# CVPR23/Depth-guided-Texture-Diffusion-for-Image-Semantic-Segmentation

Measured on NVIDIA B200. Metric: rgbd_images_per_sec_384, higher is better.
Workload: dtype bf16

## Files before the change

depth-guided-texture-diffusion-for-image-semantic-segmentation_b200/csrc/blackwell.cuh:

```cuda
#pragma once
#include <cuda.h>
#include <cuda_runtime.h>
#include <stdint.h>
#include <stdio.h>

namespace dgtd {
namespace bw {

__device__ __forceinline__ uint32_t smem_u32(const void* p) {
  return static_cast<uint32_t>(__cvta_generic_to_shared(p));
}

__device__ __forceinline__ bool elect_one() {
  uint32_t pred = 0;
  asm volatile(
      "{\n\t.reg .pred p;\n\t"
      "elect.sync _|p, 0xffffffff;\n\t"
      "selp.u32 %0, 1, 0, p;\n\t}"
      : "=r"(pred));
  return pred != 0;
}

__device__ __forceinline__ void mbar_init(uint64_t* bar, uint32_t count) {
  asm volatile("mbarrier.init.shared::cta.b64 [%0], %1;" ::"r"(smem_u32(bar)), "r"(count));
// ... 155 lines not shown
  asm volatile(
      "tcgen05.ld.sync.aligned.32x32b.x32.b32 "
      "{%0, %1, %2, %3, %4, %5, %6, %7, %8, %9, %10, %11, %12, %13, %14, %15, "
      "%16, %17, %18, %19, %20, %21, %22, %23, %24, %25, %26, %27, %28, %29, %30, %31}, [%32];"
      : "=r"(v[0]), "=r"(v[1]), "=r"(v[2]), "=r"(v[3]), "=r"(v[4]), "=r"(v[5]), "=r"(v[6]), "=r"(v[7]),
        "=r"(v[8]), "=r"(v[9]), "=r"(v[10]), "=r"(v[11]), "=r"(v[12]), "=r"(v[13]), "=r"(v[14]),
        "=r"(v[15]), "=r"(v[16]), "=r"(v[17]), "=r"(v[18]), "=r"(v[19]), "=r"(v[20]), "=r"(v[21]),
        "=r"(v[22]), "=r"(v[23]), "=r"(v[24]), "=r"(v[25]), "=r"(v[26]), "=r"(v[27]), "=r"(v[28]),
        "=r"(v[29]), "=r"(v[30]), "=r"(v[31])
      : "r"(taddr)
      : "memory");
}
__device__ __forceinline__ void tmem_ld_wait() { asm volatile("tcgen05.wait::ld.sync.aligned;" ::: "memory"); }

__device__ __forceinline__ uint64_t umma_smem_desc_kmajor(uint32_t smem_addr, uint32_t row_bytes) {
  const uint64_t layout = row_bytes == 128 ? 2ull : row_bytes == 64 ? 4ull : 6ull;
  return (uint64_t)((smem_addr >> 4) & 0x3FFF) | ((uint64_t)((8 * row_bytes) >> 4) << 32) |
         (1ull << 46) | (layout << 61);
}
__device__ __forceinline__ uint64_t umma_smem_desc_mnmajor_sw128(uint32_t smem_addr, uint32_t lbo_bytes,
                                                                 uint32_t sbo_bytes) {
  return (uint64_t)((smem_addr >> 4) & 0x3FFF) | ((uint64_t)((lbo_bytes >> 4) & 0x3FFF) << 16) |
         ((uint64_t)((sbo_bytes >> 4) & 0x3FFF) << 32) | (1ull << 46) | (2ull << 61);
}
__host__ __device__ constexpr uint32_t umma_idesc_bf16(int M, int N) {
  return (1u << 4) | (1u << 7) | (1u << 10) | ((uint32_t)(N >> 3) << 17) | ((uint32_t)(M >> 4) << 24);
}
__host__ __device__ constexpr uint32_t umma_idesc_tf32(int M, int N) {
  return (1u << 4) | (2u << 7) | (2u << 10) | ((uint32_t)(N >> 3) << 17) | ((uint32_t)(M >> 4) << 24);
}

}

typedef CUresult (*PFN_tmapEncodeTiled)(CUtensorMap*, CUtensorMapDataType, cuuint32_t, void*,
                                        const cuuint64_t*, const cuuint64_t*, const cuuint32_t*,
                                        const cuuint32_t*, CUtensorMapInterleave, CUtensorMapSwizzle,
                                        CUtensorMapL2promotion, CUtensorMapFloatOOBfill);
PFN_tmapEncodeTiled get_tmap_encoder();

int make_tmap(CUtensorMap* out, const void* base, CUtensorMapDataType dt, int rank,
              const uint64_t* dims, const uint64_t* strides_bytes, const uint32_t* box,
              CUtensorMapSwizzle swz);

}
```

depth-guided-texture-diffusion-for-image-semantic-segmentation_b200/csrc/mlp_fused.cu:

```cuda
#include "tc_common.cuh"

namespace dgtd {

namespace mlpf {

constexpr int C = 128, HID = 4 * C, HC = 128, NCH = HID / HC;
constexpr int BLK = 128 * 64 * 2;
constexpr int KB1 = C / 64, KB2 = HC / 64;
constexpr int A_BYTES = KB1 * BLK, H_BYTES = KB2 * BLK;
constexpr int WST = 4;
constexpr int NEPI = 16;
constexpr int STG_BYTES = NEPI * 4096;
constexpr int OFF_A = 0, OFF_H = A_BYTES, OFF_W = OFF_H + 2 * H_BYTES, OFF_STG = OFF_W + WST * BLK, OFF_BAR = OFF_STG + STG_BYTES;
constexpr int NBARS = 2 + 2 * WST + 4 + 4 + 4 + NEPI;
constexpr int SMEM = OFF_BAR + NBARS * 8 + 16;
constexpr int THREADS = 128 + NEPI * 32;
static_assert(SMEM <= 232448, "shared memory budget");

struct Params {
  const float* row_stats;
  const float* col_s;
  const float* cbias;
  const float* b2;
  const float* gamma;
  const float* res;
  float* out;
  int M, tiles;
};

__device__ __forceinline__ uint32_t swz_l(int lane) { return (uint32_t)(lane & 7); }

__global__ void __launch_bounds__(THREADS, 1)
mlp_fused_kernel(const __grid_constant__ CUtensorMap tmY, const __grid_constant__ CUtensorMap tmW1,
                 const __grid_constant__ CUtensorMap tmW2, const __grid_constant__ CUtensorMap tmRes,
                 const __grid_constant__ CUtensorMap tmOut, const Params p) {
  extern __shared__ __align__(1024) uint8_t smem[];
  uint8_t* sA = smem + OFF_A;
  uint8_t* sH = smem + OFF_H;
  uint8_t* sW = smem + OFF_W;
  uint64_t* bars = reinterpret_cast<uint64_t*>(smem + OFF_BAR);
  uint8_t* sStg = smem + OFF_STG;
  uint64_t* a_full = bars;
  uint64_t* a_empty = a_full + 1;
  uint64_t* w_full = a_empty + 1;
  uint64_t* w_empty = w_full + WST;
  uint64_t* c1_full = w_empty + WST;
  uint64_t* c1_empty = c1_full + 2;
  uint64_t* h_full = c1_empty + 2;
  uint64_t* h_empty = h_full + 2;
  uint64_t* c2_full = h_empty + 2;
  uint64_t* c2_empty = c2_full + 2;
  uint64_t* r_full = c2_empty + 2;
  uint32_t* tmem_slot = reinterpret_cast<uint32_t*>(r_full + NEPI);

  const int warp = threadIdx.x >> 5, lane = threadIdx.x & 31;
  if (warp == 0 && lane == 0) {
    bw::prefetch_tmap(&tmY);
    bw::prefetch_tmap(&tmW1);
    bw::prefetch_tmap(&tmW2);
    bw::prefetch_tmap(&tmRes);
    bw::prefetch_tmap(&tmOut);
  }
  if (warp == 1 && lane == 0) {
    bw::mbar_init(a_full, 1);
    bw::mbar_init(a_empty, 1);
    for (int i = 0; i < 2; ++i) {
      bw::mbar_init(&c1_full[i], 1);
      bw::mbar_init(&c1_empty[i], NEPI);
      bw::mbar_init(&h_full[i], NEPI);
      bw::mbar_init(&h_empty[i], 1);
      bw::mbar_init(&c2_full[i], 1);
      bw::mbar_init(&c2_empty[i], NEPI);
    }
    for (int i = 0; i < NEPI; ++i) bw::mbar_init(&r_full[i], 1);
    for (int i = 0; i < WST; ++i) {
      bw::mbar_init(&w_full[i], 1);
      bw::mbar_init(&w_empty[i], 1);
    }
    bw::fence_mbar_init();
  }
  if (warp == 2) bw::tmem_alloc(tmem_slot, 512);
  bw::tc_fence_before();
  __syncthreads();
  bw::tc_fence_after();
  const uint32_t tmem_base = *tmem_slot;

  if (warp == 0) {
    if (lane == 0) {
      int ws = 0;
      uint32_t wph = 0;
      auto load_w = [&](const CUtensorMap* tm, int k0, int r0) {
        bw::mbar_wait(&w_empty[ws], wph ^ 1);
        bw::mbar_arrive_expect_tx(&w_full[ws], BLK);
        bw::tma_load_2d(tm, &w_full[ws], sW + ws * BLK, k0, r0);
        if (++ws == WST) { ws = 0; wph ^= 1; }
      };
      int it = 0;
      for (int tile = blockIdx.x; tile < p.tiles; tile += gridDim.x, ++it) {
        bw::mbar_wait(a_empty, (it & 1) ^ 1);
        bw::mbar_arrive_expect_tx(a_full, A_BYTES);
        for (int kb = 0; kb < KB1; ++kb) bw::tma_load_2d(&tmY, a_full, sA + kb * BLK, kb * 64, tile * 128);
        for (int s = 0; s <= NCH; ++s) {
          if (s < NCH)
            for (int kb = 0; kb < KB1; ++kb) load_w(&tmW1, kb * 64, s * HC);
          if (s >= 1)
            for (int kb = 0; kb < KB2; ++kb) load_w(&tmW2, (s - 1) * HC + kb * 64, 0);
        }
      }
    }
  } else if (warp == 1) {
    if (lane == 0) {
      constexpr uint32_t idesc = bw::umma_idesc_bf16(128, 128);
      int ws = 0;
      uint32_t wph = 0;
      uint32_t q1 = 0, q2 = 0;
      int it = 0;
      for (int tile = blockIdx.x; tile < p.tiles; tile += gridDim.x, ++it) {
        const int ab = it & 1;
        bw::mbar_wait(a_full, it & 1);
        for (int s = 0; s <= NCH; ++s) {
          if (s < NCH) {
            const uint32_t b = q1 & 1;
            bw::mbar_wait(&c1_empty[b], ((q1 >> 1) & 1) ^ 1);
            bw::tc_fence_after();
            const uint32_t d = tmem_base + b * HC;
            for (int kb = 0; kb < KB1; ++kb) {
              bw::mbar_wait(&w_full[ws], wph);
              bw::tc_fence_after();
              const uint64_t da = bw::umma_smem_desc_kmajor(bw::smem_u32(sA + kb * BLK), 128);
              const uint64_t db = bw::umma_smem_desc_kmajor(bw::smem_u32(sW + ws * BLK), 128);
#pragma unroll
              for (int k = 0; k < 4; ++k) bw::umma_bf16(d, da + 2 * k, db + 2 * k, idesc, (kb | k) != 0);
              bw::umma_commit(&w_empty[ws]);
              if (++ws == WST) { ws = 0; wph ^= 1; }
            }
            bw::umma_commit(&c1_full[b]);
            if (s == NCH - 1) bw::umma_commit(a_empty);
            ++q1;
          }
          if (s >= 1) {
            const int c = s - 1;
            const uint32_t b = q2 & 1;
            if (c == 0) {
              bw::mbar_wait(&c2_empty[ab], ((it >> 1) & 1) ^ 1);
              bw::tc_fence_after();
            }
            bw::mbar_wait(&h_full[b], (q2 >> 1) & 1);
            bw::tc_fence_after();
            const uint32_t d = tmem_base + 2 * HC + ab * C;
            for (int kb = 0; kb < KB2; ++kb) {
              bw::mbar_wait(&w_full[ws], wph);
              bw::tc_fence_after();
              const uint64_t da = bw::umma_smem_desc_kmajor(bw::smem_u32(sH + b * H_BYTES + kb * BLK), 128);
              const uint64_t db = bw::umma_smem_desc_kmajor(bw::smem_u32(sW + ws * BLK), 128);
#pragma unroll
              for (int k = 0; k < 4; ++k) bw::umma_bf16(d, da + 2 * k, db + 2 * k, idesc, (c | kb | k) != 0);
              bw::umma_commit(&w_empty[ws]);
              if (++ws == WST) { ws = 0; wph ^= 1; }
            }
            bw::umma_commit(&h_empty[b]);
            if (c == NCH - 1) bw::umma_commit(&c2_full[ab]);
            ++q2;
          }
        }
      }
    }
  } else if (warp >= 4) {
    const int quad = warp & 3, part = (warp - 4) >> 2, ew = warp - 4;
    const int r = quad * 32 + lane;
    const uint32_t lane_addr = (uint32_t)(quad * 32) << 16;
    uint8_t* hrow_p = sH + (part >> 1) * BLK + r * 128;
    const uint32_t swz = (uint32_t)(r & 7);
    uint8_t* stg = sStg + ew * 4096;
    uint8_t* srow_p = stg + lane * 128;
    uint64_t* rbar = &r_full[ew];
    uint32_t q = 0;
    int it = 0;
    for (int tile = blockIdx.x; tile < p.tiles; tile += gridDim.x, ++it) {
      const int ab = it & 1;
      const int row0 = tile * 128 + quad * 32;
      if (lane == 0) {
        bw::tma_store_wait_read<0>();
        bw::mbar_arrive_expect_tx(rbar, 4096);
        bw::tma_load_2d(&tmRes, rbar, stg, part * 32, row0);
      }
      const float2 rs = __ldg(reinterpret_cast<const float2*>(p.row_stats) + row0 + lane);
      const uint64_t nm = pk2(-rs.x, -rs.x), rr = pk2(rs.y, rs.y);
      for (int c = 0; c < NCH; ++c, ++q) {
        const uint32_t b = q & 1;
        bw::mbar_wait(&c1_full[b], (q >> 1) & 1);
        bw::tc_fence_after();
        uint32_t v[32];
        bw::tmem_ld_32x32(tmem_base + lane_addr + b * HC + part * 32, v);
        bw::tmem_ld_wait();
        bw::tc_fence_before();
        __syncwarp();
        if (lane == 0) bw::mbar_arrive(&c1_empty[b]);
        bw::mbar_wait(&h_empty[b], ((q >> 1) & 1) ^ 1);
        const int n0 = c * HC + part * 32;
#pragma unroll
        for (int j = 0; j < 32; j += 8) {
          const float4 s0 = __ldg(reinterpret_cast<const float4*>(p.col_s + n0 + j));
          const float4 s1 = __ldg(reinterpret_cast<const float4*>(p.col_s + n0 + j + 4));
          const float4 b0 = __ldg(reinterpret_cast<const float4*>(p.cbias + n0 + j));
          const float4 b1 = __ldg(reinterpret_cast<const float4*>(p.cbias + n0 + j + 4));
          float f[8];
#pragma unroll
          for (int e = 0; e < 8; ++e) f[e] = __uint_as_float(v[j + e]);
          uint64_t x0 = fma2(nm, pk2(s0.x, s0.y), pk2(f[0], f[1])), x1 = fma2(nm, pk2(s0.z, s0.w), pk2(f[2], f[3]));
          uint64_t x2 = fma2(nm, pk2(s1.x, s1.y), pk2(f[4], f[5])), x3 = fma2(nm, pk2(s1.z, s1.w), pk2(f[6], f[7]));
          up2(fma2(rr, x0, pk2(b0.x, b0.y)), f[0], f[1]);
          up2(fma2(rr, x1, pk2(b0.z, b0.w)), f[2], f[3]);
          up2(fma2(rr, x2, pk2(b1.x, b1.y)), f[4], f[5]);
          up2(fma2(rr, x3, pk2(b1.z, b1.w)), f[6], f[7]);
#pragma unroll
          for (int e = 0; e < 8; e += 2) DGTD_GELU2(f[e], f[e + 1]);
          const __nv_bfloat162 a0 = __floats2bfloat162_rn(f[0], f[1]), a1 = __floats2bfloat162_rn(f[2], f[3]);
          const __nv_bfloat162 a2 = __floats2bfloat162_rn(f[4], f[5]), a3 = __floats2bfloat162_rn(f[6], f[7]);
          const uint32_t ch = (uint32_t)((part & 1) * 4 + (j >> 3));
          *reinterpret_cast<uint4*>(hrow_p + b * H_BYTES + ((ch ^ swz) << 4)) =
              make_uint4(*reinterpret_cast<const uint32_t*>(&a0), *reinterpret_cast<const uint32_t*>(&a1),
                         *reinterpret_cast<const uint32_t*>(&a2), *reinterpret_cast<const uint32_t*>(&a3));
        }
        bw::fence_proxy_async_smem();
        __syncwarp();
        if (lane == 0) bw::mbar_arrive(&h_full[b]);
      }
      bw::mbar_wait(&c2_full[ab], (it >> 1) & 1);
      bw::tc_fence_after();
      uint32_t v[32];
      bw::tmem_ld_32x32(tmem_base + lane_addr + 2 * HC + ab * C + part * 32, v);
      bw::tmem_ld_wait();
      bw::tc_fence_before();
      __syncwarp();
      if (lane == 0) bw::mbar_arrive(&c2_empty[ab]);
      bw::mbar_wait(rbar, it & 1);
#pragma unroll
      for (int j = 0; j < 32; j += 4) {
        float4* sp = reinterpret_cast<float4*>(srow_p + ((((uint32_t)(j >> 2)) ^ swz_l(lane)) << 4));
        float4 x = *sp;
        const float4 bb = __ldg(reinterpret_cast<const float4*>(p.b2 + part * 32 + j));
        float4 g = make_float4(1.f, 1.f, 1.f, 1.f);
        if (p.gamma) g = __ldg(reinterpret_cast<const float4*>(p.gamma + part * 32 + j));
        x.x += g.x * (__uint_as_float(v[j]) + bb.x);
        x.y += g.y * (__uint_as_float(v[j + 1]) + bb.y);
        x.z += g.z * (__uint_as_float(v[j + 2]) + bb.z);
        x.w += g.w * (__uint_as_float(v[j + 3]) + bb.w);
        *sp = x;
      }
      bw::fence_proxy_async_smem();
      __syncwarp();
      if (lane == 0) {
        bw::tma_store_2d(&tmOut, stg, part * 32, row0);
        bw::tma_store_commit();
      }
    }
    if (lane == 0) bw::tma_store_wait_all<0>();
  }

  bw::tc_fence_before();
  __syncthreads();
  if (warp == 2) {
    bw::tc_fence_after();
    bw::tmem_dealloc(tmem_base, 512);
  }
}

}
}

using namespace dgtd;

extern "C" int dgtd_convnext_mlp_fused_fwd(const void* y, const float* row_stats, const void* w1, const float* col_s,
                                           const float* cbias, const void* w2, const float* b2, const float* gamma,
                                           const float* residual, float* out, int64_t M, int C, dgtd_stream_t stream) {
  using namespace mlpf;
  DGTD_CHECK_ARG(y && row_stats && w1 && col_s && cbias && w2 && b2 && residual && out, "convnext_mlp_fused: null pointer");
  DGTD_CHECK_ARG(C == mlpf::C, "convnext_mlp_fused: C = %d is not built (stage 0, C = 128, only)", C);
  DGTD_CHECK_ARG(M > 0 && M % 128 == 0 && M < ((int64_t)1 << 31), "convnext_mlp_fused: M = %lld must be a positive multiple of 128",
                 (long long)M);
  cudaStream_t s = (cudaStream_t)stream;
  CUtensorMap tmY, tmW1, tmW2;
  {
    uint64_t dims[2] = {(uint64_t)C, (uint64_t)M}, str[1] = {(uint64_t)C * 2};
    uint32_t box[2] = {64, 128};
    if (make_tmap(&tmY, y, CU_TENSOR_MAP_DATA_TYPE_BFLOAT16, 2, dims, str, box, CU_TENSOR_MAP_SWIZZLE_128B)) return -3;
  }
  {
    uint64_t dims[2] = {(uint64_t)C, (uint64_t)HID}, str[1] = {(uint64_t)C * 2};
    uint32_t box[2] = {64, 128};
    if (make_tmap(&tmW1, w1, CU_TENSOR_MAP_DATA_TYPE_BFLOAT16, 2, dims, str, box, CU_TENSOR_MAP_SWIZZLE_128B)) return -3;
  }
  {
    uint64_t dims[2] = {(uint64_t)HID, (uint64_t)C}, str[1] = {(uint64_t)HID * 2};
    uint32_t box[2] = {64, 128};
    if (make_tmap(&tmW2, w2, CU_TENSOR_MAP_DATA_TYPE_BFLOAT16, 2, dims, str, box, CU_TENSOR_MAP_SWIZZLE_128B)) return -3;
  }
  CUtensorMap tmRes, tmOut;
  {
    uint64_t dims[2] = {(uint64_t)C, (uint64_t)M}, str[1] = {(uint64_t)C * 4};
    uint32_t box[2] = {32, 32};
    if (make_tmap(&tmRes, residual, CU_TENSOR_MAP_DATA_TYPE_FLOAT32, 2, dims, str, box, CU_TENSOR_MAP_SWIZZLE_128B)) return -3;
    if (make_tmap(&tmOut, out, CU_TENSOR_MAP_DATA_TYPE_FLOAT32, 2, dims, str, box, CU_TENSOR_MAP_SWIZZLE_128B)) return -3;
  }
  static bool configured = false;
  if (!configured) {
    cudaError_t e = cudaFuncSetAttribute(mlp_fused_kernel, cudaFuncAttributeMaxDynamicSharedMemorySize, SMEM);
    if (e != cudaSuccess) {
      set_error("convnext_mlp_fused: cannot opt in to %d B of shared memory: %s", SMEM, cudaGetErrorString(e));
      return -2;
    }
    configured = true;
  }
  Params p;
  p.row_stats = row_stats; p.col_s = col_s; p.cbias = cbias; p.b2 = b2; p.gamma = gamma; p.res = residual; p.out = out;
  p.M = (int)M; p.tiles = (int)(M / 128);
  const int grid = p.tiles < sm_count() ? p.tiles : sm_count();
  mlp_fused_kernel<<<grid, THREADS, SMEM, s>>>(tmY, tmW1, tmW2, tmRes, tmOut, p);
  DGTD_LAUNCH_CHECK("convnext_mlp_fused");
  return 0;
}
```

depth-guided-texture-diffusion-for-image-semantic-segmentation_b200/csrc/tc_gemm2.cu:

```cuda
#include "tc_common.cuh"

namespace dgtd {

namespace bw2 {
__device__ __forceinline__ uint32_t cta_rank() {
  uint32_t r;
  asm volatile("mov.u32 %0, %%cluster_ctarank;" : "=r"(r));
  return r;
}
__device__ __forceinline__ void cluster_sync() {
  asm volatile("barrier.cluster.arrive.release.aligned;" ::: "memory");
  asm volatile("barrier.cluster.wait.acquire.aligned;" ::: "memory");
}
__device__ __forceinline__ uint32_t map_to_rank(const void* p, uint32_t rank) {
  uint32_t r;
  asm volatile("mapa.shared::cluster.u32 %0, %1, %2;" : "=r"(r) : "r"(bw::smem_u32(p)), "r"(rank));
  return r;
}
__device__ __forceinline__ void mbar_arrive_cluster(uint32_t cluster_addr) {
  asm volatile("mbarrier.arrive.shared::cluster.b64 _, [%0];" ::"r"(cluster_addr) : "memory");
}
__device__ __forceinline__ void tma_load_2d_2sm(const CUtensorMap* m, uint32_t leader_bar, void* dst, int c0,
                                                int c1) {
  asm volatile(
      "cp.async.bulk.tensor.2d.cta_group::2.shared::cluster.global.mbarrier::complete_tx::bytes [%0], [%1, {%3, %4}], [%2];"
      ::"r"(bw::smem_u32(dst)), "l"(reinterpret_cast<uint64_t>(m)), "r"(leader_bar), "r"(c0), "r"(c1)
      : "memory");
}
__device__ __forceinline__ void tmem_alloc_2sm(uint32_t* dst_smem, uint32_t cols) {
  asm volatile("tcgen05.alloc.cta_group::2.sync.aligned.shared::cta.b32 [%0], %1;" ::"r"(bw::smem_u32(dst_smem)),
               "r"(cols)
               : "memory");
  asm volatile("tcgen05.relinquish_alloc_permit.cta_group::2.sync.aligned;" ::: "memory");
}
__device__ __forceinline__ void tmem_dealloc_2sm(uint32_t addr, uint32_t cols) {
  asm volatile("tcgen05.dealloc.cta_group::2.sync.aligned.b32 %0, %1;" ::"r"(addr), "r"(cols) : "memory");
}
__device__ __forceinline__ void umma_bf16_2sm(uint32_t tmem_d, uint64_t da, uint64_t db, uint32_t idesc,
                                              uint32_t accumulate) {
  asm volatile(
      "{\n\t.reg .pred p;\n\t"
      "setp.ne.b32 p, %4, 0;\n\t"
      "tcgen05.mma.cta_group::2.kind::f16 [%0], %1, %2, %3, p;\n\t}"
      ::"r"(tmem_d), "l"(da), "l"(db), "r"(idesc), "r"(accumulate)
      : "memory");
}
__device__ __forceinline__ void umma_commit_2sm(uint64_t* bar) {
  asm volatile(
      "tcgen05.commit.cta_group::2.mbarrier::arrive::one.shared::cluster.multicast::cluster.b64 [%0], %1;"
      ::"r"(bw::smem_u32(bar)), "h"((uint16_t)3)
      : "memory");
}
}

template <int BN>
struct Tc2Cfg {
  static constexpr int BM = 128, BK = 64;
  static constexpr int A_BYTES = BM * BK * 2, B_BYTES = (BN / 2) * BK * 2;
  static constexpr int STAGES = BN >= 256 ? 5 : 6;
  static constexpr int TMEM_COLS = 2 * BN;
  static constexpr int STG_BYTES = 8 * 2 * 4096;
  static constexpr int XCH_BYTES = BN == 128 ? 2 * 8 * 32 * 8 : 0;
  static constexpr int SMEM_BYTES = STAGES * (A_BYTES + B_BYTES) + STG_BYTES + 512 + XCH_BYTES + 1024;
};

template <int BN, int ACT, typename OT, bool RESIDUAL, int NEPI = 8, bool LNROW = false>
__global__ void __cluster_dims__(2, 1, 1) __launch_bounds__(128 + 32 * NEPI, 1)
tc_gemm2_kernel(const __grid_constant__ CUtensorMap tmA, const __grid_constant__ CUtensorMap tmB,
                const __grid_constant__ CUtensorMap tmOut, const __grid_constant__ CUtensorMap tmRes,
                const TcParams p) {
  using Cfg = Tc2Cfg<BN>;
  constexpr int BM = Cfg::BM, BK = Cfg::BK, STAGES = Cfg::STAGES;
  extern __shared__ __align__(1024) uint8_t smem[];
  uint8_t* sA = smem;
  uint8_t* sB = smem + STAGES * Cfg::A_BYTES;
  uint8_t* sStg = smem + STAGES * (Cfg::A_BYTES + Cfg::B_BYTES);
  uint64_t* bars = reinterpret_cast<uint64_t*>(sStg + Cfg::STG_BYTES);
  uint64_t* rbars = bars + 2 * STAGES + 6;
  uint64_t* full = bars;
  uint64_t* empty = bars + STAGES;
  uint64_t* tfull = bars + 2 * STAGES;
  uint64_t* tempty = bars + 2 * STAGES + 2;
  uint32_t* tmem_slot = reinterpret_cast<uint32_t*>(bars + 2 * STAGES + 4);

  const int warp = threadIdx.x >> 5, lane = threadIdx.x & 31;
  const uint32_t rank = bw2::cta_rank();
// ... 245 lines not shown
```

depth-guided-texture-diffusion-for-image-semantic-segmentation_b200/twig/ops/functions/texture_diffusion_func.py:

```python
from __future__ import annotations

from typing import List, Optional, Sequence, Tuple

import torch
from torch.autograd import Function
from torch.autograd.function import once_differentiable

from .. import capi
from ..capi import ACT_GELU, ACT_NONE, ACT_RELU, BF16, F32, call, check_cuda, ptr, stream

__all__ = [
    "surface_normals", "HighpassPlan", "fft_highpass", "diffusion_front", "MessagePassingFunction",
    "message_passing_core", "message_passing_tiled", "conv1x1_nchw_autograd", "resize_bilinear_nchw_autograd", "conv1x1_nchw", "resize_nchw", "layer_norm",
    "stem", "stem_patches", "ln_rows_", "fusion_sum", "ln_patchify", "dwconv7_ln", "dwconv7_ln_tma", "linear", "linear_ln", "linear_tf32", "linear_residual_", "conv_nhwc", "conv_nhwc_grouped",
    "resize_nhwc", "cast", "nhwc_to_nchw", "nchw_to_nhwc", "enable_gemm_profile", "collect_gemm_profile",
]


_PROFILE = {"on": False, "events": []}


def enable_gemm_profile(on: bool = True):
    _PROFILE["on"] = bool(on)
    _PROFILE["events"] = []
# ... 351 lines not shown
    M = a.numel() // K
    N = w.shape[0]
    assert w.shape[1] == K and a.dtype == torch.bfloat16 and w.dtype == torch.bfloat16 and a.is_contiguous()
    out = torch.empty(tuple(a.shape[:-1]) + (N,), device=a.device, dtype=torch.float32)
    call("dgtd_linear_ln_fwd", ptr(a), ptr(w), ptr(bias), ptr(ln_w), ptr(ln_b), float(eps), ptr(out), M, N, K, stream())
    return out


def linear_tf32(a: torch.Tensor, w: torch.Tensor, bias: Optional[torch.Tensor]) -> torch.Tensor:
    check_cuda(a, w, bias)
    K = a.shape[-1]
    M = a.numel() // K
    N = w.shape[0]
    assert w.shape[1] == K and a.dtype == torch.float32 and w.dtype == torch.float32 and a.is_contiguous()
    out = torch.empty(tuple(a.shape[:-1]) + (N,), device=a.device, dtype=torch.float32)
    call("dgtd_linear_tf32_fwd", ptr(a), ptr(w), ptr(bias), ptr(out), M, N, K, N, stream())
    return out


def linear_residual_(a: torch.Tensor, w: torch.Tensor, bias, gamma, keep: Optional[torch.Tensor],
                     rows_per_sample: int, residual: torch.Tensor, out: Optional[torch.Tensor] = None):
    check_cuda(a, w, bias, gamma, keep, residual)
    K = a.shape[-1]
    M = a.numel() // K
    N = w.shape[0]
    assert residual.dtype == torch.float32 and residual.numel() == M * N
    out = residual if out is None else out
    with _timed(2.0 * M * N * K, a.dtype == torch.bfloat16, (M, N, K)):
        call("dgtd_linear_residual_fwd", ptr(a), ptr(w), ptr(bias), ptr(gamma), ptr(keep), rows_per_sample,
             ptr(residual), ptr(out), M, N, K, capi.dtype_code(a.dtype), stream())
    return out


MLP_FUSED_C = (128,)


def convnext_mlp_fused_(y: torch.Tensor, row_stats: torch.Tensor, w1: torch.Tensor, col_s: torch.Tensor,
                        cbias: torch.Tensor, w2: torch.Tensor, b2: torch.Tensor, gamma: Optional[torch.Tensor],
                        residual: torch.Tensor, out: Optional[torch.Tensor] = None) -> torch.Tensor:
    check_cuda(y, row_stats, w1, col_s, cbias, w2, b2, gamma, residual)
    C = y.shape[-1]
    M = y.numel() // C
    assert y.dtype == torch.bfloat16 and w1.dtype == torch.bfloat16 and w2.dtype == torch.bfloat16
    assert w1.shape == (4 * C, C) and w2.shape == (C, 4 * C) and row_stats.shape == (M, 2)
    assert residual.dtype == torch.float32 and residual.numel() == M * C
    out = residual if out is None else out
    with _timed(4.0 * M * C * 4 * C, True, (M, 4 * C, C)):
        call("dgtd_convnext_mlp_fused_fwd", ptr(y), ptr(row_stats), ptr(w1), ptr(col_s), ptr(cbias), ptr(w2), ptr(b2),
             ptr(gamma), ptr(residual), ptr(out), M, C, stream())
    return out


def fusion_sum(levels: List[torch.Tensor], hw: List[Tuple[int, int]], bias, B: int, want_nhwc=True,
               want_nchw=False, pad_to: int = 0):
    check_cuda(*levels, bias)
    C = levels[0].shape[-1]
    dev = levels[0].device
    h0, w0 = hw[0]
    nhwc = torch.empty(B, h0, w0, C, device=dev, dtype=torch.float32) if want_nhwc else None
    nchw = torch.empty(B, C, h0, w0, device=dev, dtype=torch.float32) if want_nchw else None
    pad = torch.empty(B, h0, w0, pad_to, device=dev, dtype=torch.bfloat16) if pad_to else None
    hw_arr = (capi.c_int * 8)(*[v for pair in hw for v in pair])
    call("dgtd_fusion_sum_fwd", ptr(levels[0]), ptr(levels[1]), ptr(levels[2]), ptr(levels[3]), hw_arr,
         ptr(bias), ptr(nhwc), ptr(nchw), ptr(pad), pad_to, B, C, stream())
    return nhwc, nchw, pad


# ... 82 lines not shown
```

Measured before the change: 5303.

## Convert fused ConvNeXt MLP kernel to 2-SM cluster UMMA and add C=256

Rewrites the fused ConvNeXt MLP kernel to run as 2-CTA clusters using cta_group::2 tcgen05 MMAs with M=256 tiles, splitting weight tiles across the pair of CTAs. It double-buffers the A tile and C2 accumulators for C=128 and reworks the epilogue staging and residual handling. It also templates the kernel over C and enables the fused path for C=256 stages, so more of the network uses the fused kernel. The cluster barriers and cross-CTA signalling add synchronisation complexity and carry correctness risk.

After: 5222, median of 6. -1.5%, worse.

```diff
diff --git a/depth-guided-texture-diffusion-for-image-semantic-segmentation_b200/csrc/blackwell.cuh b/depth-guided-texture-diffusion-for-image-semantic-segmentation_b200/csrc/blackwell.cuh
--- a/depth-guided-texture-diffusion-for-image-semantic-segmentation_b200/csrc/blackwell.cuh
+++ b/depth-guided-texture-diffusion-for-image-semantic-segmentation_b200/csrc/blackwell.cuh
@@ -211,6 +211,60 @@
 
 }
 
+namespace bw2 {
+__device__ __forceinline__ uint32_t cta_rank() {
+  uint32_t r;
+  asm volatile("mov.u32 %0, %%cluster_ctarank;" : "=r"(r));
+  return r;
+}
+__device__ __forceinline__ void cluster_sync() {
+  asm volatile("barrier.cluster.arrive.release.aligned;" ::: "memory");
+  asm volatile("barrier.cluster.wait.acquire.aligned;" ::: "memory");
+}
+__device__ __forceinline__ uint32_t map_to_rank(const void* p, uint32_t rank) {
+  uint32_t r;
+  asm volatile("mapa.shared::cluster.u32 %0, %1, %2;" : "=r"(r) : "r"(bw::smem_u32(p)), "r"(rank));
+  return r;
+}
+__device__ __forceinline__ void mbar_arrive_cluster(uint32_t cluster_addr) {
+  asm volatile("mbarrier.arrive.shared::cluster.b64 _, [%0];" ::"r"(cluster_addr) : "memory");
+}
+__device__ __forceinline__ void mbar_arrive_cluster_release(uint32_t cluster_addr) {
+  asm volatile("mbarrier.arrive.release.cluster.shared::cluster.b64 _, [%0];" ::"r"(cluster_addr) : "memory");
+}
+__device__ __forceinline__ void tma_load_2d_2sm(const CUtensorMap* m, uint32_t leader_bar, void* dst, int c0,
+                                                int c1) {
+  asm volatile(
+      "cp.async.bulk.tensor.2d.cta_group::2.shared::cluster.global.mbarrier::complete_tx::bytes [%0], [%1, {%3, %4}], [%2];"
+      ::"r"(bw::smem_u32(dst)), "l"(reinterpret_cast<uint64_t>(m)), "r"(leader_bar), "r"(c0), "r"(c1)
+      : "memory");
+}
+__device__ __forceinline__ void tmem_alloc_2sm(uint32_t* dst_smem, uint32_t cols) {
+  asm volatile("tcgen05.alloc.cta_group::2.sync.aligned.shared::cta.b32 [%0], %1;" ::"r"(bw::smem_u32(dst_smem)),
+               "r"(cols)
+               : "memory");
+  asm volatile("tcgen05.relinquish_alloc_permit.cta_group::2.sync.aligned;" ::: "memory");
+}
+__device__ __forceinline__ void tmem_dealloc_2sm(uint32_t addr, uint32_t cols) {
+  asm volatile("tcgen05.dealloc.cta_group::2.sync.aligned.b32 %0, %1;" ::"r"(addr), "r"(cols) : "memory");
+}
+__device__ __forceinline__ void umma_bf16_2sm(uint32_t tmem_d, uint64_t da, uint64_t db, uint32_t idesc,
+                                              uint32_t accumulate) {
+  asm volatile(
+      "{\n\t.reg .pred p;\n\t"
+      "setp.ne.b32 p, %4, 0;\n\t"
+      "tcgen05.mma.cta_group::2.kind::f16 [%0], %1, %2, %3, p;\n\t}"
+      ::"r"(tmem_d), "l"(da), "l"(db), "r"(idesc), "r"(accumulate)
+      : "memory");
+}
+__device__ __forceinline__ void umma_commit_2sm(uint64_t* bar) {
+  asm volatile(
+      "tcgen05.commit.cta_group::2.mbarrier::arrive::one.shared::cluster.multicast::cluster.b64 [%0], %1;"
+      ::"r"(bw::smem_u32(bar)), "h"((uint16_t)3)
+      : "memory");
+}
+}
+
 typedef CUresult (*PFN_tmapEncodeTiled)(CUtensorMap*, CUtensorMapDataType, cuuint32_t, void*,
                                         const cuuint64_t*, const cuuint64_t*, const cuuint32_t*,
                                         const cuuint32_t*, CUtensorMapInterleave, CUtensorMapSwizzle,
diff --git a/depth-guided-texture-diffusion-for-image-semantic-segmentation_b200/csrc/mlp_fused.cu b/depth-guided-texture-diffusion-for-image-semantic-segmentation_b200/csrc/mlp_fused.cu
--- a/depth-guided-texture-diffusion-for-image-semantic-segmentation_b200/csrc/mlp_fused.cu
+++ b/depth-guided-texture-diffusion-for-image-semantic-segmentation_b200/csrc/mlp_fused.cu
@@ -4,18 +4,31 @@
 
 namespace mlpf {
 
-constexpr int C = 128, HID = 4 * C, HC = 128, NCH = HID / HC;
-constexpr int BLK = 128 * 64 * 2;
-constexpr int KB1 = C / 64, KB2 = HC / 64;
-constexpr int A_BYTES = KB1 * BLK, H_BYTES = KB2 * BLK;
-constexpr int WST = 4;
-constexpr int NEPI = 16;
-constexpr int STG_BYTES = NEPI * 4096;
-constexpr int OFF_A = 0, OFF_H = A_BYTES, OFF_W = OFF_H + 2 * H_BYTES, OFF_STG = OFF_W + WST * BLK, OFF_BAR = OFF_STG + STG_BYTES;
-constexpr int NBARS = 2 + 2 * WST + 4 + 4 + 4 + NEPI;
-constexpr int SMEM = OFF_BAR + NBARS * 8 + 16;
-constexpr int THREADS = 128 + NEPI * 32;
-static_assert(SMEM <= 232448, "shared memory budget");
+template <int C>
+struct Cfg {
+  static constexpr int HID = 4 * C, HC = 128, NCH = HID / HC;
+  static constexpr int BLK = 128 * 64 * 2;
+  static constexpr int KB1 = C / 64, KB2 = HC / 64;
+  static constexpr int A_BYTES = KB1 * BLK, H_BYTES = KB2 * BLK;
+  static constexpr int NA = C == 128 ? 2 : 1;
+  static constexpr int NACC2 = C == 128 ? 2 : 1;
+  static constexpr int WST = 4, SLOT = 16384;
+  static constexpr int W1_HALF = 64 * 64 * 2;
+  static constexpr int W2_HALF = (C / 2) * 64 * 2;
+  static constexpr int W2_PER_SLOT = SLOT / W2_HALF;
+  static constexpr int SLOTS1 = KB1 / 2, SLOTS2 = KB2 / W2_PER_SLOT;
+  static constexpr int NEPI = 16;
+  static constexpr int CW = C / 4;
+  static constexpr int STG = 2048;
+  static constexpr int OFF_A = 0, OFF_H = NA * A_BYTES, OFF_W = OFF_H + 2 * H_BYTES, OFF_STG = OFF_W + WST * SLOT;
+  static constexpr int OFF_BAR = OFF_STG + NEPI * STG;
+  static constexpr int NBARS = 2 * NA + 2 * WST + 4 + 4 + 2 * NACC2;
+  static constexpr int SMEM = OFF_BAR + NBARS * 8 + 16;
+  static constexpr int THREADS = 128 + NEPI * 32;
+  static_assert(SMEM <= 232448, "shared memory budget");
+  static_assert(SLOTS1 * 2 == KB1 && SLOTS2 * W2_PER_SLOT == KB2, "weight blocks fill whole ring slots");
+  static_assert(2 * HC + NACC2 * C <= 512, "TMEM budget");
+};
 
 struct Params {
   const float* row_stats;
@@ -24,64 +37,69 @@
   const float* b2;
   const float* gamma;
   const float* res;
-  float* out;
   int M, tiles;
 };
 
-__device__ __forceinline__ uint32_t swz_l(int lane) { return (uint32_t)(lane & 7); }
-
-__global__ void __launch_bounds__(THREADS, 1)
+template <int C>
+__global__ void __cluster_dims__(2, 1, 1) __launch_bounds__(Cfg<C>::THREADS, 1)
 mlp_fused_kernel(const __grid_constant__ CUtensorMap tmY, const __grid_constant__ CUtensorMap tmW1,
-                 const __grid_constant__ CUtensorMap tmW2, const __grid_constant__ CUtensorMap tmRes,
-                 const __grid_constant__ CUtensorMap tmOut, const Params p) {
+                 const __grid_constant__ CUtensorMap tmW2, const __grid_constant__ CUtensorMap tmOut, const Params p) {
+  using K = Cfg<C>;
+  constexpr int HC = K::HC, NCH = K::NCH, NA = K::NA, NACC2 = K::NACC2, WST = K::WST, NEPI = K::NEPI, CW = K::CW;
   extern __shared__ __align__(1024) uint8_t smem[];
-  uint8_t* sA = smem + OFF_A;
-  uint8_t* sH = smem + OFF_H;
-  uint8_t* sW = smem + OFF_W;
-  uint64_t* bars = reinterpret_cast<uint64_t*>(smem + OFF_BAR);
-  uint8_t* sStg = smem + OFF_STG;
+  uint8_t* sA = smem + K::OFF_A;
+  uint8_t* sH = smem + K::OFF_H;
+  uint8_t* sW = smem + K::OFF_W;
+  uint8_t* sStg = smem + K::OFF_STG;
+  uint64_t* bars = reinterpret_cast<uint64_t*>(smem + K::OFF_BAR);
   uint64_t* a_full = bars;
-  uint64_t* a_empty = a_full + 1;
-  uint64_t* w_full = a_empty + 1;
+  uint64_t* a_empty = a_full + NA;
+  uint64_t* w_full = a_empty + NA;
   uint64_t* w_empty = w_full + WST;
   uint64_t* c1_full = w_empty + WST;
   uint64_t* c1_empty = c1_full + 2;
   uint64_t* h_full = c1_empty + 2;
   uint64_t* h_empty = h_full + 2;
   uint64_t* c2_full = h_empty + 2;
-  uint64_t* c2_empty = c2_full + 2;
-  uint64_t* r_full = c2_empty + 2;
-  uint32_t* tmem_slot = reinterpret_cast<uint32_t*>(r_full + NEPI);
+  uint64_t* c2_empty = c2_full + NACC2;
+  uint32_t* tmem_slot = reinterpret_cast<uint32_t*>(c2_empty + NACC2);
 
   const int warp = threadIdx.x >> 5, lane = threadIdx.x & 31;
+  const uint32_t rank = bw2::cta_rank();
+  const bool leader = rank == 0;
+  const int cluster_id = blockIdx.x >> 1, num_clusters = gridDim.x >> 1;
+
+  bw2::cluster_sync();
   if (warp == 0 && lane == 0) {
     bw::prefetch_tmap(&tmY);
     bw::prefetch_tmap(&tmW1);
     bw::prefetch_tmap(&tmW2);
-    bw::prefetch_tmap(&tmRes);
     bw::prefetch_tmap(&tmOut);
   }
   if (warp == 1 && lane == 0) {
-    bw::mbar_init(a_full, 1);
-    bw::mbar_init(a_empty, 1);
+    for (int i = 0; i < NA; ++i) {
+      bw::mbar_init(&a_full[i], 2);
+      bw::mbar_init(&a_empty[i], 1);
+    }
+    for (int i = 0; i < WST; ++i) {
+      bw::mbar_init(&w_full[i], 2);
+      bw::mbar_init(&w_empty[i], 1);
+    }
     for (int i = 0; i < 2; ++i) {
       bw::mbar_init(&c1_full[i], 1);
-      bw::mbar_init(&c1_empty[i], NEPI);
-      bw::mbar_init(&h_full[i], NEPI);
+      bw::mbar_init(&c1_empty[i], 2 * NEPI);
+      bw::mbar_init(&h_full[i], 2 * NEPI);
       bw::mbar_init(&h_empty[i], 1);
+    }
+    for (int i = 0; i < NACC2; ++i) {
       bw::mbar_init(&c2_full[i], 1);
-      bw::mbar_init(&c2_empty[i], NEPI);
-    }
-    for (int i = 0; i < NEPI; ++i) bw::mbar_init(&r_full[i], 1);
-    for (int i = 0; i < WST; ++i) {
-      bw::mbar_init(&w_full[i], 1);
-      bw::mbar_init(&w_empty[i], 1);
+      bw::mbar_init(&c2_empty[i], 2 * NEPI);
     }
     bw::fence_mbar_init();
   }
-  if (warp == 2) bw::tmem_alloc(tmem_slot, 512);
+  if (warp == 2) bw2::tmem_alloc_2sm(tmem_slot, 512);
   bw::tc_fence_before();
-  __syncthreads();
+  bw2::cluster_sync();
   bw::tc_fence_after();
   const uint32_t tmem_base = *tmem_slot;
 
@@ -89,77 +107,104 @@
     if (lane == 0) {
       int ws = 0;
       uint32_t wph = 0;
-      auto load_w = [&](const CUtensorMap* tm, int k0, int r0) {
+      auto slot = [&]() -> uint32_t {
         bw::mbar_wait(&w_empty[ws], wph ^ 1);
-        bw::mbar_arrive_expect_tx(&w_full[ws], BLK);
-        bw::tma_load_2d(tm, &w_full[ws], sW + ws * BLK, k0, r0);
-        if (++ws == WST) { ws = 0; wph ^= 1; }
+        const uint32_t lbar = bw2::map_to_rank(&w_full[ws], 0);
+        if (leader) bw::mbar_arrive_expect_tx(&w_full[ws], 2 * K::SLOT);
+        else bw2::mbar_arrive_cluster(lbar);
+        return lbar;
       };
+      auto next = [&]() { if (++ws == WST) { ws = 0; wph ^= 1; } };
       int it = 0;
-      for (int tile = blockIdx.x; tile < p.tiles; tile += gridDim.x, ++it) {
-        bw::mbar_wait(a_empty, (it & 1) ^ 1);
-        bw::mbar_arrive_expect_tx(a_full, A_BYTES);
-        for (int kb = 0; kb < KB1; ++kb) bw::tma_load_2d(&tmY, a_full, sA + kb * BLK, kb * 64, tile * 128);
+      for (int tile = cluster_id; tile < p.tiles; tile += num_clusters, ++it) {
+        const int ab = it % NA;
+        bw::mbar_wait(&a_empty[ab], ((it / NA) & 1) ^ 1);
+        const uint32_t abar = bw2::map_to_rank(&a_full[ab], 0);
+        if (leader) bw::mbar_arrive_expect_tx(&a_full[ab], 2 * K::A_BYTES);
+        else bw2::mbar_arrive_cluster(abar);
+        for (int kb = 0; kb < K::KB1; ++kb)
+          bw2::tma_load_2d_2sm(&tmY, abar, sA + ab * K::A_BYTES + kb * K::BLK, kb * 64, tile * 256 + (int)rank * 128);
         for (int s = 0; s <= NCH; ++s) {
           if (s < NCH)
-            for (int kb = 0; kb < KB1; ++kb) load_w(&tmW1, kb * 64, s * HC);
+            for (int i = 0; i < K::SLOTS1; ++i) {
+              const uint32_t lbar = slot();
+              for (int j = 0; j < 2; ++j)
+                bw2::tma_load_2d_2sm(&tmW1, lbar, sW + ws * K::SLOT + j * K::W1_HALF, (2 * i + j) * 64,
+                                     s * HC + (int)rank * 64);
+              next();
+            }
           if (s >= 1)
-            for (int kb = 0; kb < KB2; ++kb) load_w(&tmW2, (s - 1) * HC + kb * 64, 0);
+            for (int i = 0; i < K::SLOTS2; ++i) {
+              const uint32_t lbar = slot();
+              for (int j = 0; j < K::W2_PER_SLOT; ++j)
+                bw2::tma_load_2d_2sm(&tmW2, lbar, sW + ws * K::SLOT + j * K::W2_HALF,
+                                     (s - 1) * HC + (i * K::W2_PER_SLOT + j) * 64, (int)rank * (C / 2));
+              next();
+            }
         }
       }
     }
   } else if (warp == 1) {
-    if (lane == 0) {
-      constexpr uint32_t idesc = bw::umma_idesc_bf16(128, 128);
+    if (leader && lane == 0) {
+      constexpr uint32_t idesc1 = bw::umma_idesc_bf16(256, HC), idesc2 = bw::umma_idesc_bf16(256, C);
       int ws = 0;
       uint32_t wph = 0;
       uint32_t q1 = 0, q2 = 0;
       int it = 0;
-      for (int tile = blockIdx.x; tile < p.tiles; tile += gridDim.x, ++it) {
-        const int ab = it & 1;
-        bw::mbar_wait(a_full, it & 1);
+      for (int tile = cluster_id; tile < p.tiles; tile += num_clusters, ++it) {
+        const int ab = it % NA, cb = it % NACC2;
+        bw::mbar_wait(&a_full[ab], (it / NA) & 1);
+        bw::tc_fence_after();
         for (int s = 0; s <= NCH; ++s) {
           if (s < NCH) {
             const uint32_t b = q1 & 1;
             bw::mbar_wait(&c1_empty[b], ((q1 >> 1) & 1) ^ 1);
             bw::tc_fence_after();
             const uint32_t d = tmem_base + b * HC;
-            for (int kb = 0; kb < KB1; ++kb) {
+            for (int i = 0; i < K::SLOTS1; ++i) {
               bw::mbar_wait(&w_full[ws], wph);
               bw::tc_fence_after();
-              const uint64_t da = bw::umma_smem_desc_kmajor(bw::smem_u32(sA + kb * BLK), 128);
-              const uint64_t db = bw::umma_smem_desc_kmajor(bw::smem_u32(sW + ws * BLK), 128);
-#pragma unroll
-              for (int k = 0; k < 4; ++k) bw::umma_bf16(d, da + 2 * k, db + 2 * k, idesc, (kb | k) != 0);
-              bw::umma_commit(&w_empty[ws]);
+#pragma unroll
+              for (int j = 0; j < 2; ++j) {
+                const int kb = 2 * i + j;
+                const uint64_t da = bw::umma_smem_desc_kmajor(bw::smem_u32(sA + ab * K::A_BYTES + kb * K::BLK), 128);
+                const uint64_t db = bw::umma_smem_desc_kmajor(bw::smem_u32(sW + ws * K::SLOT + j * K::W1_HALF), 128);
+#pragma unroll
+                for (int k = 0; k < 4; ++k) bw2::umma_bf16_2sm(d, da + 2 * k, db + 2 * k, idesc1, (kb | k) != 0);
+              }
+              bw2::umma_commit_2sm(&w_empty[ws]);
               if (++ws == WST) { ws = 0; wph ^= 1; }
             }
-            bw::umma_commit(&c1_full[b]);
-            if (s == NCH - 1) bw::umma_commit(a_empty);
+            bw2::umma_commit_2sm(&c1_full[b]);
+            if (s == NCH - 1) bw2::umma_commit_2sm(&a_empty[ab]);
             ++q1;
           }
           if (s >= 1) {
             const int c = s - 1;
             const uint32_t b = q2 & 1;
             if (c == 0) {
-              bw::mbar_wait(&c2_empty[ab], ((it >> 1) & 1) ^ 1);
+              bw::mbar_wait(&c2_empty[cb], ((it / NACC2) & 1) ^ 1);
               bw::tc_fence_after();
             }
             bw::mbar_wait(&h_full[b], (q2 >> 1) & 1);
             bw::tc_fence_after();
-            const uint32_t d = tmem_base + 2 * HC + ab * C;
-            for (int kb = 0; kb < KB2; ++kb) {
+            const uint32_t d = tmem_base + 2 * HC + cb * C;
+            for (int i = 0; i < K::SLOTS2; ++i) {
               bw::mbar_wait(&w_full[ws], wph);
               bw::tc_fence_after();
-              const uint64_t da = bw::umma_smem_desc_kmajor(bw::smem_u32(sH + b * H_BYTES + kb * BLK), 128);
-              const uint64_t db = bw::umma_smem_desc_kmajor(bw::smem_u32(sW + ws * BLK), 128);
-#pragma unroll
-              for (int k = 0; k < 4; ++k) bw::umma_bf16(d, da + 2 * k, db + 2 * k, idesc, (c | kb | k) != 0);
-              bw::umma_commit(&w_empty[ws]);
+#pragma unroll
+              for (int j = 0; j < K::W2_PER_SLOT; ++j) {
+                const int kb = i * K::W2_PER_SLOT + j;
+                const uint64_t da = bw::umma_smem_desc_kmajor(bw::smem_u32(sH + b * K::H_BYTES + kb * K::BLK), 128);
+                const uint64_t db = bw::umma_smem_desc_kmajor(bw::smem_u32(sW + ws * K::SLOT + j * K::W2_HALF), 128);
+#pragma unroll
+                for (int k = 0; k < 4; ++k) bw2::umma_bf16_2sm(d, da + 2 * k, db + 2 * k, idesc2, (c | kb | k) != 0);
+              }
+              bw2::umma_commit_2sm(&w_empty[ws]);
               if (++ws == WST) { ws = 0; wph ^= 1; }
             }
-            bw::umma_commit(&h_empty[b]);
-            if (c == NCH - 1) bw::umma_commit(&c2_full[ab]);
+            bw2::umma_commit_2sm(&h_empty[b]);
+            if (c == NCH - 1) bw2::umma_commit_2sm(&c2_full[cb]);
             ++q2;
           }
         }
@@ -169,25 +214,28 @@
     const int quad = warp & 3, part = (warp - 4) >> 2, ew = warp - 4;
     const int r = quad * 32 + lane;
     const uint32_t lane_addr = (uint32_t)(quad * 32) << 16;
-    uint8_t* hrow_p = sH + (part >> 1) * BLK + r * 128;
+    uint8_t* hrow_p = sH + (part >> 1) * K::BLK + r * 128;
     const uint32_t swz = (uint32_t)(r & 7);
-    uint8_t* stg = sStg + ew * 4096;
-    uint8_t* srow_p = stg + lane * 128;
-    uint64_t* rbar = &r_full[ew];
+    uint8_t* stg = sStg + ew * K::STG;
+    uint8_t* srow_p = stg + lane * 64;
+    const uint32_t sswz = (uint32_t)((lane >> 1) & 3);
+    const uint32_t c1e = bw2::map_to_rank(c1_empty, 0), hf = bw2::map_to_rank(h_full, 0);
+    const uint32_t c2e = bw2::map_to_rank(c2_empty, 0);
     uint32_t q = 0;
     int it = 0;
-    for (int tile = blockIdx.x; tile < p.tiles; tile += gridDim.x, ++it) {
-      const int ab = it & 1;
-      const int row0 = tile * 128 + quad * 32;
-      if (lane == 0) {
-        bw::tma_store_wait_read<0>();
-        bw::mbar_arrive_expect_tx(rbar, 4096);
-        bw::tma_load_2d(&tmRes, rbar, stg, part * 32, row0);
-      }
-      const float2 rs = __ldg(reinterpret_cast<const float2*>(p.row_stats) + row0 + lane);
+    for (int tile = cluster_id; tile < p.tiles; tile += num_clusters, ++it) {
+      const int cb = it % NACC2;
+      const int row0 = tile * 256 + (int)rank * 128 + quad * 32;
+      const int row = row0 + lane;
+      const bool valid = row < p.M;
+      const float2 rs = valid ? __ldg(reinterpret_cast<const float2*>(p.row_stats) + row) : make_float2(0.f, 0.f);
       const uint64_t nm = pk2(-rs.x, -rs.x), rr = pk2(rs.y, rs.y);
+      const float* resrow = p.res + (size_t)(valid ? row : 0) * C + part * CW;
       for (int c = 0; c < NCH; ++c, ++q) {
         const uint32_t b = q & 1;
+        if (c == NCH - 1 && valid)
+#pragma unroll
+          for (int l = 0; l < CW * 4; l += 128) asm volatile("prefetch.global.L2 [%0];" ::"l"(resrow + l / 4));
         bw::mbar_wait(&c1_full[b], (q >> 1) & 1);
         bw::tc_fence_after();
         uint32_t v[32];
@@ -195,7 +243,7 @@
         bw::tmem_ld_wait();
         bw::tc_fence_before();
         __syncwarp();
-        if (lane == 0) bw::mbar_arrive(&c1_empty[b]);
+        if (lane == 0) bw2::mbar_arrive_cluster(c1e + 8 * b);
         bw::mbar_wait(&h_empty[b], ((q >> 1) & 1) ^ 1);
         const int n0 = c * HC + part * 32;
 #pragma unroll
@@ -218,52 +266,107 @@
           const __nv_bfloat162 a0 = __floats2bfloat162_rn(f[0], f[1]), a1 = __floats2bfloat162_rn(f[2], f[3]);
           const __nv_bfloat162 a2 = __floats2bfloat162_rn(f[4], f[5]), a3 = __floats2bfloat162_rn(f[6], f[7]);
           const uint32_t ch = (uint32_t)((part & 1) * 4 + (j >> 3));
-          *reinterpret_cast<uint4*>(hrow_p + b * H_BYTES + ((ch ^ swz) << 4)) =
+          *reinterpret_cast<uint4*>(hrow_p + b * K::H_BYTES + ((ch ^ swz) << 4)) =
               make_uint4(*reinterpret_cast<const uint32_t*>(&a0), *reinterpret_cast<const uint32_t*>(&a1),
                          *reinterpret_cast<const uint32_t*>(&a2), *reinterpret_cast<const uint32_t*>(&a3));
         }
         bw::fence_proxy_async_smem();
         __syncwarp();
-        if (lane == 0) bw::mbar_arrive(&h_full[b]);
+        if (lane == 0) bw2::mbar_arrive_cluster_release(hf + 8 * b);
       }
-      bw::mbar_wait(&c2_full[ab], (it >> 1) & 1);
-      bw::tc_fence_after();
-      uint32_t v[32];
-      bw::tmem_ld_32x32(tmem_base + lane_addr + 2 * HC + ab * C + part * 32, v);
-      bw::tmem_ld_wait();
-      bw::tc_fence_before();
-      __syncwarp();
-      if (lane == 0) bw::mbar_arrive(&c2_empty[ab]);
-      bw::mbar_wait(rbar, it & 1);
-#pragma unroll
-      for (int j = 0; j < 32; j += 4) {
-        float4* sp = reinterpret_cast<float4*>(srow_p + ((((uint32_t)(j >> 2)) ^ swz_l(lane)) << 4));
-        float4 x = *sp;
-        const float4 bb = __ldg(reinterpret_cast<const float4*>(p.b2 + part * 32 + j));
-        float4 g = make_float4(1.f, 1.f, 1.f, 1.f);
-        if (p.gamma) g = __ldg(reinterpret_cast<const float4*>(p.gamma + part * 32 + j));
-        x.x += g.x * (__uint_as_float(v[j]) + bb.x);
-        x.y += g.y * (__uint_as_float(v[j + 1]) + bb.y);
-        x.z += g.z * (__uint_as_float(v[j + 2]) + bb.z);
-        x.w += g.w * (__uint_as_float(v[j + 3]) + bb.w);
-        *sp = x;
+#pragma unroll 1
+      for (int g = 0; g < CW / 32; ++g) {
+        float4 x[8];
+#pragma unroll
+        for (int j = 0; j < 8; ++j)
+          x[j] = valid ? reinterpret_cast<const float4*>(resrow + g * 32)[j] : make_float4(0.f, 0.f, 0.f, 0.f);
+        if (g == 0) {
+          bw::mbar_wait(&c2_full[cb], (it / NACC2) & 1);
+          bw::tc_fence_after();
+        }
+        uint32_t v[32];
+        bw::tmem_ld_32x32(tmem_base + lane_addr + 2 * HC + cb * C + part * CW + g * 32, v);
+        bw::tmem_ld_wait();
+        if (g == CW / 32 - 1) {
+          bw::tc_fence_before();
+          __syncwarp();
+          if (lane == 0) bw2::mbar_arrive_cluster(c2e + 8 * cb);
+        }
+#pragma unroll
+        for (int h = 0; h < 2; ++h) {
+          if (lane == 0) bw::tma_store_wait_read<0>();
+          __syncwarp();
+#pragma unroll
+          for (int jj = 0; jj < 4; ++jj) {
+            const int j = h * 4 + jj, col = part * CW + g * 32 + 4 * j;
+            const float4 bb = __ldg(reinterpret_cast<const float4*>(p.b2 + col));
+            float4 gm = make_float4(1.f, 1.f, 1.f, 1.f);
+            if (p.gamma) gm = __ldg(reinterpret_cast<const float4*>(p.gamma + col));
+            float4 o = x[j];
+            o.x += gm.x * (__uint_as_float(v[4 * j]) + bb.x);
+            o.y += gm.y * (__uint_as_float(v[4 * j + 1]) + bb.y);
+            o.z += gm.z * (__uint_as_float(v[4 * j + 2]) + bb.z);
+            o.w += gm.w * (__uint_as_float(v[4 * j + 3]) + bb.w);
+            *reinterpret_cast<float4*>(srow_p + (((uint32_t)jj ^ sswz) << 4)) = o;
+          }
+          bw::fence_proxy_async_smem();
+          __syncwarp();
+          if (lane == 0) {
+            bw::tma_store_2d(&tmOut, stg, part * CW + g * 32 + h * 16, row0);
+            bw::tma_store_commit();
+          }
+        }
       }
-      bw::fence_proxy_async_smem();
-      __syncwarp();
-      if (lane == 0) {
-        bw::tma_store_2d(&tmOut, stg, part * 32, row0);
-        bw::tma_store_commit();
-      }
     }
     if (lane == 0) bw::tma_store_wait_all<0>();
   }
 
   bw::tc_fence_before();
-  __syncthreads();
+  bw2::cluster_sync();
   if (warp == 2) {
     bw::tc_fence_after();
-    bw::tmem_dealloc(tmem_base, 512);
-  }
+    bw2::tmem_dealloc_2sm(tmem_base, 512);
+  }
+}
+
+template <int C>
+static int launch(const void* y, const void* w1, const void* w2, float* out, Params p, cudaStream_t s) {
+  using K = Cfg<C>;
+  CUtensorMap tmY, tmW1, tmW2, tmOut;
+  {
+    uint64_t dims[2] = {(uint64_t)C, (uint64_t)p.M}, str[1] = {(uint64_t)C * 2};
+    uint32_t box[2] = {64, 128};
+    if (make_tmap(&tmY, y, CU_TENSOR_MAP_DATA_TYPE_BFLOAT16, 2, dims, str, box, CU_TENSOR_MAP_SWIZZLE_128B)) return -3;
+  }
+  {
+    uint64_t dims[2] = {(uint64_t)C, (uint64_t)K::HID}, str[1] = {(uint64_t)C * 2};
+    uint32_t box[2] = {64, 64};
+    if (make_tmap(&tmW1, w1, CU_TENSOR_MAP_DATA_TYPE_BFLOAT16, 2, dims, str, box, CU_TENSOR_MAP_SWIZZLE_128B)) return -3;
+  }
+  {
+    uint64_t dims[2] = {(uint64_t)K::HID, (uint64_t)C}, str[1] = {(uint64_t)K::HID * 2};
+    uint32_t box[2] = {64, (uint32_t)(C / 2)};
+    if (make_tmap(&tmW2, w2, CU_TENSOR_MAP_DATA_TYPE_BFLOAT16, 2, dims, str, box, CU_TENSOR_MAP_SWIZZLE_128B)) return -3;
+  }
+  {
+    uint64_t dims[2] = {(uint64_t)C, (uint64_t)p.M}, str[1] = {(uint64_t)C * 4};
+    uint32_t box[2] = {16, 32};
+    if (make_tmap(&tmOut, out, CU_TENSOR_MAP_DATA_TYPE_FLOAT32, 2, dims, str, box, CU_TENSOR_MAP_SWIZZLE_64B)) return -3;
+  }
+  static bool configured = false;
+  if (!configured) {
+    cudaError_t e = cudaFuncSetAttribute(mlp_fused_kernel<C>, cudaFuncAttributeMaxDynamicSharedMemorySize, K::SMEM);
+    if (e != cudaSuccess) {
+      set_error("convnext_mlp_fused: cannot opt in to %d B of shared memory: %s", K::SMEM, cudaGetErrorString(e));
+      return -2;
+    }
+    configured = true;
+  }
+  const int pairs = sm_count() / 2;
+  const int clusters = p.tiles < pairs ? p.tiles : pairs;
+  mlp_fused_kernel<C><<<2 * clusters, K::THREADS, K::SMEM, s>>>(tmY, tmW1, tmW2, tmOut, p);
+  DGTD_LAUNCH_CHECK("convnext_mlp_fused");
+  return 0;
 }
 
 }
@@ -276,47 +379,14 @@
                                            const float* residual, float* out, int64_t M, int C, dgtd_stream_t stream) {
   using namespace mlpf;
   DGTD_CHECK_ARG(y && row_stats && w1 && col_s && cbias && w2 && b2 && residual && out, "convnext_mlp_fused: null pointer");
-  DGTD_CHECK_ARG(C == mlpf::C, "convnext_mlp_fused: C = %d is not built (stage 0, C = 128, only)", C);
+  DGTD_CHECK_ARG(C == 128 || C == 256, "convnext_mlp_fused: C = %d is not built (C = 128, 256 only)", C);
   DGTD_CHECK_ARG(M > 0 && M % 128 == 0 && M < ((int64_t)1 << 31), "convnext_mlp_fused: M = %lld must be a positive multiple of 128",
                  (long long)M);
+  DGTD_CHECK_ARG(out == residual || out + M * C <= residual || residual + M * C <= out,
+                 "convnext_mlp_fused: out must be residual or not overlap it");
+  Params p;
+  p.row_stats = row_stats; p.col_s = col_s; p.cbias = cbias; p.b2 = b2; p.gamma = gamma; p.res = residual;
+  p.M = (int)M; p.tiles = (int)((M + 255) / 256);
   cudaStream_t s = (cudaStream_t)stream;
-  CUtensorMap tmY, tmW1, tmW2;
-  {
-    uint64_t dims[2] = {(uint64_t)C, (uint64_t)M}, str[1] = {(uint64_t)C * 2};
-    uint32_t box[2] = {64, 128};
-    if (make_tmap(&tmY, y, CU_TENSOR_MAP_DATA_TYPE_BFLOAT16, 2, dims, str, box, CU_TENSOR_MAP_SWIZZLE_128B)) return -3;
-  }
-  {
-    uint64_t dims[2] = {(uint64_t)C, (uint64_t)HID}, str[1] = {(uint64_t)C * 2};
-    uint32_t box[2] = {64, 128};
-    if (make_tmap(&tmW1, w1, CU_TENSOR_MAP_DATA_TYPE_BFLOAT16, 2, dims, str, box, CU_TENSOR_MAP_SWIZZLE_128B)) return -3;
-  }
-  {
-    uint64_t dims[2] = {(uint64_t)HID, (uint64_t)C}, str[1] = {(uint64_t)HID * 2};
-    uint32_t box[2] = {64, 128};
-    if (make_tmap(&tmW2, w2, CU_TENSOR_MAP_DATA_TYPE_BFLOAT16, 2, dims, str, box, CU_TENSOR_MAP_SWIZZLE_128B)) return -3;
-  }
-  CUtensorMap tmRes, tmOut;
-  {
-    uint64_t dims[2] = {(uint64_t)C, (uint64_t)M}, str[1] = {(uint64_t)C * 4};
-    uint32_t box[2] = {32, 32};
-    if (make_tmap(&tmRes, residual, CU_TENSOR_MAP_DATA_TYPE_FLOAT32, 2, dims, str, box, CU_TENSOR_MAP_SWIZZLE_128B)) return -3;
-    if (make_tmap(&tmOut, out, CU_TENSOR_MAP_DATA_TYPE_FLOAT32, 2, dims, str, box, CU_TENSOR_MAP_SWIZZLE_128B)) return -3;
-  }
-  static bool configured = false;
-  if (!configured) {
-    cudaError_t e = cudaFuncSetAttribute(mlp_fused_kernel, cudaFuncAttributeMaxDynamicSharedMemorySize, SMEM);
-    if (e != cudaSuccess) {
-      set_error("convnext_mlp_fused: cannot opt in to %d B of shared memory: %s", SMEM, cudaGetErrorString(e));
-      return -2;
-    }
-    configured = true;
-  }
-  Params p;
-  p.row_stats = row_stats; p.col_s = col_s; p.cbias = cbias; p.b2 = b2; p.gamma = gamma; p.res = residual; p.out = out;
-  p.M = (int)M; p.tiles = (int)(M / 128);
-  const int grid = p.tiles < sm_count() ? p.tiles : sm_count();
-  mlp_fused_kernel<<<grid, THREADS, SMEM, s>>>(tmY, tmW1, tmW2, tmRes, tmOut, p);
-  DGTD_LAUNCH_CHECK("convnext_mlp_fused");
-  return 0;
-}
+  return C == 128 ? launch<128>(y, w1, w2, out, p, s) : launch<256>(y, w1, w2, out, p, s);
+}
diff --git a/depth-guided-texture-diffusion-for-image-semantic-segmentation_b200/csrc/tc_gemm2.cu b/depth-guided-texture-diffusion-for-image-semantic-segmentation_b200/csrc/tc_gemm2.cu
--- a/depth-guided-texture-diffusion-for-image-semantic-segmentation_b200/csrc/tc_gemm2.cu
+++ b/depth-guided-texture-diffusion-for-image-semantic-segmentation_b200/csrc/tc_gemm2.cu
@@ -1,57 +1,6 @@
 #include "tc_common.cuh"
 
 namespace dgtd {
-
-namespace bw2 {
-__device__ __forceinline__ uint32_t cta_rank() {
-  uint32_t r;
-  asm volatile("mov.u32 %0, %%cluster_ctarank;" : "=r"(r));
-  return r;
-}
-__device__ __forceinline__ void cluster_sync() {
-  asm volatile("barrier.cluster.arrive.release.aligned;" ::: "memory");
-  asm volatile("barrier.cluster.wait.acquire.aligned;" ::: "memory");
-}
-__device__ __forceinline__ uint32_t map_to_rank(const void* p, uint32_t rank) {
-  uint32_t r;
-  asm volatile("mapa.shared::cluster.u32 %0, %1, %2;" : "=r"(r) : "r"(bw::smem_u32(p)), "r"(rank));
-  return r;
-}
-__device__ __forceinline__ void mbar_arrive_cluster(uint32_t cluster_addr) {
-  asm volatile("mbarrier.arrive.shared::cluster.b64 _, [%0];" ::"r"(cluster_addr) : "memory");
-}
-__device__ __forceinline__ void tma_load_2d_2sm(const CUtensorMap* m, uint32_t leader_bar, void* dst, int c0,
-                                                int c1) {
-  asm volatile(
-      "cp.async.bulk.tensor.2d.cta_group::2.shared::cluster.global.mbarrier::complete_tx::bytes [%0], [%1, {%3, %4}], [%2];"
-      ::"r"(bw::smem_u32(dst)), "l"(reinterpret_cast<uint64_t>(m)), "r"(leader_bar), "r"(c0), "r"(c1)
-      : "memory");
-}
-__device__ __forceinline__ void tmem_alloc_2sm(uint32_t* dst_smem, uint32_t cols) {
-  asm volatile("tcgen05.alloc.cta_group::2.sync.aligned.shared::cta.b32 [%0], %1;" ::"r"(bw::smem_u32(dst_smem)),
-               "r"(cols)
-               : "memory");
-  asm volatile("tcgen05.relinquish_alloc_permit.cta_group::2.sync.aligned;" ::: "memory");
-}
-__device__ __forceinline__ void tmem_dealloc_2sm(uint32_t addr, uint32_t cols) {
-  asm volatile("tcgen05.dealloc.cta_group::2.sync.aligned.b32 %0, %1;" ::"r"(addr), "r"(cols) : "memory");
-}
-__device__ __forceinline__ void umma_bf16_2sm(uint32_t tmem_d, uint64_t da, uint64_t db, uint32_t idesc,
-                                              uint32_t accumulate) {
-  asm volatile(
-      "{\n\t.reg .pred p;\n\t"
-      "setp.ne.b32 p, %4, 0;\n\t"
-      "tcgen05.mma.cta_group::2.kind::f16 [%0], %1, %2, %3, p;\n\t}"
-      ::"r"(tmem_d), "l"(da), "l"(db), "r"(idesc), "r"(accumulate)
-      : "memory");
-}
-__device__ __forceinline__ void umma_commit_2sm(uint64_t* bar) {
-  asm volatile(
-      "tcgen05.commit.cta_group::2.mbarrier::arrive::one.shared::cluster.multicast::cluster.b64 [%0], %1;"
-      ::"r"(bw::smem_u32(bar)), "h"((uint16_t)3)
-      : "memory");
-}
-}
 
 template <int BN>
 struct Tc2Cfg {
diff --git a/depth-guided-texture-diffusion-for-image-semantic-segmentation_b200/twig/ops/functions/texture_diffusion_func.py b/depth-guided-texture-diffusion-for-image-semantic-segmentation_b200/twig/ops/functions/texture_diffusion_func.py
--- a/depth-guided-texture-diffusion-for-image-semantic-segmentation_b200/twig/ops/functions/texture_diffusion_func.py
+++ b/depth-guided-texture-diffusion-for-image-semantic-segmentation_b200/twig/ops/functions/texture_diffusion_func.py
@@ -407,7 +407,7 @@
     return out
 
 
-MLP_FUSED_C = (128,)
+MLP_FUSED_C = (128, 256)
 
 
 def convnext_mlp_fused_(y: torch.Tensor, row_stats: torch.Tensor, w1: torch.Tensor, col_s: torch.Tensor,
```
